# Microtelecom/libperseus-sdr

Hardware: AMD Instinct MI355X
Metric: input MS/s through unpack+decimate, 1/2/4/8 GPU; % HBM-roofline (higher is better)
Workload: dtype i8xi8->i32, f32 out

## Files before the change

### libperseus-sdr_amd/csrc/ddc_kernels.h

```cpp
#ifndef PDDC_DDC_KERNELS_H
#define PDDC_DDC_KERNELS_H

#include <hip/hip_runtime.h>
#include <stdint.h>

#include <atomic>

namespace pddc {

enum InFmt { IN_PACKED24 = 0, IN_F32C = 1 };

struct Tunables {
    std::atomic<int> fir8_dyn_pct{ -1 };
    std::atomic<int> fir8_chunk{ 0 };
    std::atomic<int> fir8_walk{ -1 };
    std::atomic<int> gen_shape_nt{ 0 }, gen_shape_p{ 0 };
    std::atomic<int> no_firp{ 0 };
    std::atomic<int> firp_packed_p{ 0 };
    std::atomic<int> unpack_blocks{ 512 };
    std::atomic<int> debug{ 0 };
    std::atomic<int> push_three_streams{ 0 }, gang_copy_out{ 0 }, gang_gen_inline{ 0 }, gang_solo{ 0 };
    std::atomic<int> chan_run{ 0 };
    std::atomic<int> wblank_run{ 0 };
    std::atomic<int> wblank_chunk{ 0 };
};
Tunables &tunables();
bool set_tunable(const char *name, int value);
bool get_tunable(const char *name, int *value);

struct NcoArgs {
    unsigned long long n0 = 0;
    uint32_t freg = 0;
    uint32_t phase_off = 0;
    uint32_t freg_hist = 0;
    float    lo_c[8], lo_s[8];
    float    lo_c_hist[8], lo_s_hist[8];
};
void nco_fill_steps(NcoArgs *a);

struct Fir8Stage3 {
    const float *taps = nullptr;
    const void  *hist = nullptr;
    void        *hist_out = nullptr;
    float       *out = nullptr;
    void        *seam = nullptr;
    unsigned    *flags = nullptr;
    long long    n_out = 0;
    int d = 0, ntaps = 0, h = 0;
    int off = 0;
    int g = 0, ng = 0;
    int spl = 0, seglen = 0, sl = 0;
    int padf = 0;
    int seam_stride = 0;
};

struct GenTail {
    const float *in = nullptr;
    const float *hist = nullptr;
    float       *hist_out = nullptr;
    float       *out = nullptr;
    const float *taps = nullptr;
    long long    first = 0, n_out = 0, n_batch = 0;
    int          H = 0, D = 0, ntaps = 0;
    int          span = 0, a = 31;
    int          nblocks = 0;
    unsigned     lds = 0;
    int          kind = 0;
    const float *taps2 = nullptr;
    int          nbq = 0;
};
bool gen_tail_shape(GenTail *t, size_t lds_cap, bool have_taps2);
hipError_t launch_gen_tail(const GenTail &t, hipStream_t s);

struct Fir8Args {
    const void *in;
    const void *hist;
    void       *hist_out;
    float      *out;
    const float *taps_blk;
    const float *taps2_blk = nullptr;
    const void  *hist2 = nullptr;
    void        *hist2_out = nullptr;
    unsigned    *sched = nullptr;
    Fir8Stage3   s3;
    GenTail      tail;
    long long   n_in;
    NcoArgs     nco;
};
static_assert(sizeof(Fir8Args) == 448 && offsetof(Fir8Args, n_in) == 288 && offsetof(Fir8Args, nco) == 296 &&
                  offsetof(Fir8Args, nco.freg) == 304 && offsetof(Fir8Args, nco.lo_c) == 316 &&
                  offsetof(Fir8Args, nco.lo_s_hist) == 412,
              "Fir8Args: n_in, then the NCO record (8 + 12 + 128 bytes, padded to 8)");

constexpr int kFir8ManyMax = 8;
struct Fir8Many {
    Fir8Args a[kFir8ManyMax];
};
static_assert(sizeof(Fir8Many) <= 4000, "Fir8Many must fit the kernel-argument segment");
struct GenTailMany {
    GenTail t[kFir8ManyMax];
};
struct SynthMany {
    void              *dst[kFir8ManyMax];
    unsigned long long byte_offset[kFir8ManyMax];
    uint32_t           seed[kFir8ManyMax];
};
bool fir8_many_supported(int kind, int ntb, int R);
hipError_t launch_fir8_many(int kind, int ntb, int R, bool mix, const Fir8Many &m, int n, hipStream_t s);
hipError_t launch_gen_tail_many(const GenTailMany &m, int n, hipStream_t s);
hipError_t launch_synth_lcg_many(const SynthMany &m, int n, size_t nbytes, hipStream_t s);

constexpr int kFirI8Taps16Len = 128 + 6 * 64;
void fir_i8_taps16(const float *taps, int ntaps, int hist, uint16_t *out );

struct FirI8xArgs {
    const void *in;
    const void *hist;
    void       *hist_out;
    float      *out;
    const void *atab;
    long long   n_in;
    float       scale;
    float       ct[2];
    unsigned long long n0;
    uint32_t    freg, phase_off;
    const float *taps2 = nullptr;
    const void  *hist2 = nullptr;
    void        *hist2_out = nullptr;
    long long    n_out = 0;
    int          in_off = 0;
    int          hist_len = 0;
    const void  *taps16 = nullptr;
    float        two_e = 0.0f;
};
constexpr int kFirI8xTaps2Len = 2 * 68;
struct FirI8xMany {
    FirI8xArgs a[kFir8ManyMax];
};
static_assert(sizeof(FirI8xMany) <= 4000, "FirI8xMany must fit the kernel-argument segment");
int    fir_i8x_mode(int hist, bool mix);
size_t fir_i8x_table_bytes(int hist, bool mix);
bool fir_i8x_build_tables(const float *taps, int ntaps, int hist, bool mix, uint32_t freg, int8_t *tables, float *scale,
                          float ct[2], int *exp2 = nullptr);
constexpr int kFirI8xD10Hist = 64;
bool fir_i8x_d10_build_tables(const float *taps, int ntaps, int delay, uint32_t freg, int8_t *tables, float *scale, float ct[2]);
size_t fir_i8x_d10_table_bytes();
hipError_t launch_fir_i8x_d10(const FirI8xArgs &a, hipStream_t s, int max_blocks = 0, int chunk = 0, int layout = -1);
void fir_i8x_taps2(const float *taps2, int ntaps2, bool mix, uint32_t freg, float *out );
bool fir_i8x_supported(int hist, bool mix, bool fuse2);
hipError_t launch_fir_i8x_many(const FirI8xMany &m, int n, int hist, bool mix, bool fuse2, hipStream_t s, int max_blocks = 0,
                               int chunk = 0, int layout = -1);
hipError_t launch_fir_i8x(const FirI8xArgs &a, int hist, bool mix, bool fuse2, hipStream_t s, int max_blocks = 0, int chunk = 0,
                          int layout = -1 );

constexpr int kFirI8xBankMax = 4;
struct FirI8xBankCh {
    const void *atab;
    float      *out;
    void       *hist_out;
    float       scale;
    float       ct[2];
    int         hist_len;
    unsigned long long n0;
    uint32_t    freg, phase_off;
};
struct FirI8xBank {
    FirI8xArgs   a;
    FirI8xBankCh ch[kFirI8xBankMax];
};
static_assert(sizeof(FirI8xBank) <= 4000, "FirI8xBank must fit the kernel-argument segment");
static_assert(offsetof(FirI8xBankCh, n0) == 40 && sizeof(FirI8xBankCh) == 56, "hist_len sits in what was padding");
hipError_t launch_fir_i8x_bank(const FirI8xBank &b, int nch, int hist, hipStream_t s, int max_blocks = 0, int chunk = 0);
hipError_t launch_fir_i8x_bank_d10(const FirI8xBank &b, int nch, hipStream_t s, int max_blocks = 0, int chunk = 0);

constexpr float kFir8PackedTapScale = 0x1.000002p-31f;

constexpr int fir8_tile_inputs(int R, int NT = 256) { return 4 * NT * R; }
// ... 67 lines not shown
```

### libperseus-sdr_amd/csrc/ddc_kernels.hip

```cpp
#include "ddc_kernels.h"
#include "ddc_dev.h"
#include "ddc_host.h"

#include <algorithm>
#include <cmath>
#include <cstdio>
#include <cstdlib>
#include <cstring>
#include <mutex>

static constexpr int PDDC_PRIO_U = 0, PDDC_PRIO_F = 2;

namespace pddc {

Tunables &tunables()
{
    static Tunables t;
    static std::once_flag once;
    std::call_once(once, [] {
        auto env = [](const char *name, std::atomic<int> &v) {
            if (const char *e = getenv(name))
                v.store(atoi(e));
        };
        auto flag = [](const char *name, std::atomic<int> &v) {
            if (getenv(name))
                v.store(1);
        };
        env("PDDC_FIR8_DYN_PCT", t.fir8_dyn_pct);
        env("PDDC_FIR8_CHUNK", t.fir8_chunk);
        env("PDDC_FIR8_WALK", t.fir8_walk);
        if (const char *e = getenv("PDDC_GEN_SHAPE")) {
            int a = 0, b = 0;
            if (sscanf(e, "%d,%d", &a, &b) == 2) {
                t.gen_shape_nt.store(a);
                t.gen_shape_p.store(b);
            }
        }
        flag("PDDC_NO_FIRP", t.no_firp);
        env("PDDC_FIRP_PACKED_P", t.firp_packed_p);
        env("PDDC_UNPACK_BLOCKS", t.unpack_blocks);
        flag("PDDC_DEBUG", t.debug);
        flag("PDDC_PUSH_THREE_STREAMS", t.push_three_streams);
        flag("PDDC_GANG_COPY_OUT", t.gang_copy_out);
        flag("PDDC_GANG_GEN_INLINE", t.gang_gen_inline);
        flag("PDDC_GANG_SOLO", t.gang_solo);
        env("PDDC_CHAN_RUN", t.chan_run);
        env("PDDC_WBLANK_RUN", t.wblank_run);
        env("PDDC_WBLANK_CHUNK", t.wblank_chunk);
    });
    return t;
}

static std::atomic<int> *tunable_by_name(const char *name)
{
    Tunables &t = tunables();
    const struct {
        const char *n;
        std::atomic<int> *v;
    } tab[] = { { "fir8_dyn_pct", &t.fir8_dyn_pct },   { "fir8_chunk", &t.fir8_chunk },       { "fir8_walk", &t.fir8_walk },
                { "gen_shape_nt", &t.gen_shape_nt },
                { "gen_shape_p", &t.gen_shape_p },     { "no_firp", &t.no_firp },             { "firp_packed_p", &t.firp_packed_p },
                { "unpack_blocks", &t.unpack_blocks }, { "debug", &t.debug },                 { "push_three_streams", &t.push_three_streams },
                { "gang_copy_out", &t.gang_copy_out }, { "gang_gen_inline", &t.gang_gen_inline }, { "gang_solo", &t.gang_solo },
                { "chan_run", &t.chan_run },           { "wblank_run", &t.wblank_run },       { "wblank_chunk", &t.wblank_chunk } };
    if (name)
        for (const auto &e : tab)
            if (!strcmp(e.n, name))
                return e.v;
    return nullptr;
}

bool set_tunable(const char *name, int value)
{
    std::atomic<int> *v = tunable_by_name(name);
    if (v)
        v->store(value);
    return v != nullptr;
}

bool get_tunable(const char *name, int *value)
{
    std::atomic<int> *v = tunable_by_name(name);
    if (v && value)
        *value = v->load();
    return v != nullptr;
}

static constexpr int kFused3MaxChunks = 2048;
static constexpr int kPend3 = 4;

static constexpr float kUnpackScale = 0x1.000002p-31f;


__device__ __forceinline__ void unpack8_msb(const uint32_t (&w)[12], int32_t (&I)[8], int32_t (&Q)[8])
{
#pragma unroll
    for (int h = 0; h < 4; ++h) {
        const uint32_t a = w[3 * h], b = w[3 * h + 1], c = w[3 * h + 2];
        I[2 * h]     = (int32_t)__builtin_amdgcn_perm(a, a, 0x0201000cu);
        Q[2 * h]     = (int32_t)__builtin_amdgcn_perm(b, a, 0x0504030cu);
        I[2 * h + 1] = (int32_t)__builtin_amdgcn_perm(c, b, 0x0403020cu);
        Q[2 * h + 1] = (int32_t)(c & 0xffffff00u);
    }
}

template <typename P>
__device__ __forceinline__ void mix8_lo(float (&xi)[8], float (&xq)[8], float cb, float sb, const P &p)
{
#pragma unroll
    for (int e = 0; e < 8; ++e) {
        const float c = cb * p.lo_c[e] - sb * p.lo_s[e];
        const float s = cb * p.lo_s[e] + sb * p.lo_c[e];
        const float r = xi[e] * c - xq[e] * s;
        const float i = xi[e] * s + xq[e] * c;
        xi[e] = r;
        xq[e] = i;
    }
}

__device__ __forceinline__ void cmul(float &a, float &b, float c, float s)
{
    const float r = a * c - b * s;
    const float i = a * s + b * c;
    a = r;
    b = i;
}

__device__ __forceinline__ f32x2 cmul_pk(f32x2 x, f32x2 p)
{
    f32x2 t, y;
    asm("v_pk_mul_f32 %0, %1, %2 op_sel_hi:[0,1]" : "=v"(t) : "v"(x), "v"(p));
    asm("v_pk_fma_f32 %0, %1, %2, %3 op_sel:[1,1,0] op_sel_hi:[1,0,1] neg_lo:[0,1,0]" : "=v"(y) : "v"(x), "v"(p), "v"(t));
    return y;
}
__device__ __forceinline__ f32x2 cmul_pk_s(f32x2 x, float c, float s)
{
    const f32x2 t = __builtin_shufflevector(x, x, 0, 0) * f32x2{ c, s };
    return __builtin_elementwise_fma(__builtin_shufflevector(x, x, 1, 1), f32x2{ -s, c }, t);
}

__device__ __forceinline__ f32x4 cmul2(f32x4 v, float c, float s)
{
    return f32x4{ v.x * c - v.y * s, v.x * s + v.y * c, v.z * c - v.w * s, v.z * s + v.w * c };
}

template <typename P>
__device__ __forceinline__ void mix8(float (&xi)[8], float (&xq)[8], unsigned long long nabs, const P &p,
                                     uint32_t off = 0u)
{
    float cb, sb;
    nco_lo((uint32_t)nabs * p.freg + off, cb, sb);
    mix8_lo(xi, xq, cb, sb, p);
}

static void lo_steps(uint32_t freg, float *c, float *s)
{
    const double k = 6.283185307179586476925286766559 / 4294967296.0;
    for (int e = 0; e < 8; ++e) {
        const uint32_t ph = (uint32_t)((uint64_t)e * freg);
        c[e] = (float)std::cos(k * (double)ph);
        s[e] = (float)(-std::sin(k * (double)ph));
    }
}

void nco_fill_steps(NcoArgs *a)
{
    lo_steps(a->freg, a->lo_c, a->lo_s);
    lo_steps(a->freg_hist, a->lo_c_hist, a->lo_s_hist);
}

struct UnpackArgs {
    const uint8_t *in;
    void          *out;
    long long      ns;
    unsigned long long n0;
    uint32_t       freg;
    uint32_t       phase_off;
    float          lo_c[8];
    float          lo_s[8];
};

template <bool TO_I32, bool MIX>
__global__ __launch_bounds__(256) void k_unpack24(UnpackArgs p)
{
    __shared__ __attribute__((aligned(16))) uint32_t slabs[4][1024];
    const int lane = threadIdx.x & 63;
    uint32_t *slab = slabs[threadIdx.x >> 6];
    const long long ngroups = (((p.ns + 7) >> 3) + 63) & ~63LL;
    for (long long g = (long long)blockIdx.x * 256 + threadIdx.x; g < ngroups;
         g += (long long)gridDim.x * 256) {
        const long long s0 = g << 3;
        uint32_t w[12];
        if (s0 >= p.ns) {
#pragma unroll
            for (int d = 0; d < 12; ++d)
                w[d] = 0;
        } else if (s0 + 8 <= p.ns) {
            const uint4 *src = reinterpret_cast<const uint4 *>(p.in + s0 * 6);
            const uint4 a = src[0], b = src[1], c = src[2];
            w[0] = a.x; w[1] = a.y; w[2] = a.z;  w[3] = a.w;
            w[4] = b.x; w[5] = b.y; w[6] = b.z;  w[7] = b.w;
            w[8] = c.x; w[9] = c.y; w[10] = c.z; w[11] = c.w;
        } else {
            const long long nb = (p.ns - s0) * 6;
#pragma unroll
            for (int d = 0; d < 12; ++d) {
                uint32_t v = 0;
#pragma unroll
                for (int b = 0; b < 4; ++b)
                    if (4 * d + b < nb)
                        v |= (uint32_t)p.in[s0 * 6 + 4 * d + b] << (8 * b);
                w[d] = v;
            }
        }
        int32_t I[8], Q[8];
        unpack8_msb(w, I, Q);
        uint32_t o[16];
// ... 1669 lines not shown
```

### libperseus-sdr_amd/csrc/ddc_wblank.cpp

```cpp
#include "ddc_wblank.h"
#include "ddc_kernels.h"

#include <new>

using namespace pddc;

struct pddc_wblank {
    int device = 0;
    int B = 0, b = 0, H = 0, W = 0, r = 0, D = 0, TL = 0;
    uint32_t thr16 = 16, flags = 0;
    int ncu = 256;
    PackedCarry in;
    uint8_t *d_tail[3] = { nullptr, nullptr, nullptr };
    uint8_t *d_bits[3] = { nullptr, nullptr, nullptr };
    WbState *d_state[3] = { nullptr, nullptr, nullptr };
    int cur = 0;
    uint64_t *d_sums = nullptr, *d_means = nullptr;
};

static void wb_free(pddc_wblank *w)
{
    w->in.d_tail[0] = w->d_tail[0];
    w->in.d_tail[1] = w->d_tail[1];
    w->in.free();
    hipFree(w->d_tail[2]);
    for (int i = 0; i < 3; ++i) {
        hipFree(w->d_bits[i]);
        hipFree(w->d_state[i]);
    }
    hipFree(w->d_sums);
    hipFree(w->d_means);
    delete w;
}

static int wb_clear(pddc_wblank *w)
{
    WbState st{};
    for (uint64_t &h : st.hist)
        h = kWbNoBlock;
    for (int i = 0; i < 3; ++i) {
        PDDC_HIP_TRY(hipMemset(w->d_tail[i], 0, (size_t)(w->TL + 8) * 6));
        PDDC_HIP_TRY(hipMemset(w->d_bits[i], 0, (size_t)wb_tail_bit_bytes(w->D) + 16));
        PDDC_HIP_TRY(hipMemcpy(w->d_state[i], &st, sizeof st, hipMemcpyHostToDevice));
    }
    w->in.reset();
    w->in.tail_len = (uint64_t)w->TL;
    w->cur = 0;
    return PDDC_OK;
}

static int wb_create(pddc_wblank *w)
{
    PDDC_HIP_TRY(hipSetDevice(w->device));
    int ncu = 0;
    PDDC_HIP_TRY(hipDeviceGetAttribute(&ncu, hipDeviceAttributeMultiprocessorCount, w->device));
    w->ncu = ncu > 0 ? ncu : 256;
    const hipError_t e = w->in.alloc((size_t)w->TL + 8);
    w->d_tail[0] = w->in.d_tail[0];
    w->d_tail[1] = w->in.d_tail[1];
    PDDC_HIP_TRY(e);
    PDDC_HIP_TRY(hipMalloc(&w->d_tail[2], ((size_t)w->TL + 8) * 6));
    for (int i = 0; i < 3; ++i) {
        PDDC_HIP_TRY(hipMalloc(&w->d_bits[i], (size_t)wb_tail_bit_bytes(w->D) + 16));
        PDDC_HIP_TRY(hipMalloc(&w->d_state[i], sizeof(WbState)));
    }
    PDDC_HIP_TRY(hipMalloc(&w->d_sums, wblank_sums_len(w->b) * sizeof(uint64_t)));
    PDDC_HIP_TRY(hipMalloc(&w->d_means, wblank_sums_len(w->b) * sizeof(uint64_t)));
    return wb_clear(w);
}

static long long wb_chunk()
{
    const long long c = tunables().wblank_chunk.load();
    return c > 0 && c + 7 < kWbMaxChunk ? (c + 7) & ~7ll : kWbMaxChunk;
}
static long long wb_forced_run()
{
    const long long v = tunables().wblank_run.load();
    return v > 0 ? (v + kWbTile - 1) / kWbTile * kWbTile : 0;
}
static long long wb_run()
{
    const long long forced = wb_forced_run();
    return forced ? forced : kWbTile;
}

static bool wb_batch_ok(const void *p, size_t nsamples) { return !nsamples || (p && !((uintptr_t)p & 15)); }

extern "C" {

int pddc_wblank_tile_samples(void) { return kWbTile; }

int pddc_wblank_run_samples(void)
{
    const long long forced = wb_forced_run();
    return forced ? (int)(forced < (1ll << 30) ? forced : (1ll << 30)) : kWbTile;
}

int pddc_wblank_delay(const pddc_wblank *w) { return w ? w->D : 0; }

int pddc_wblank_create(pddc_wblank **out, int device, const pddc_wblank_params *params, uint32_t thr16, uint32_t flags)
{
    if (!out)
        return pddc_set_error_(PDDC_EINVAL, "null argument");
    *out = nullptr;
    if (!params)
        return pddc_set_error_(PDDC_EINVAL, "wblank: null params");
    if (!wb_params_ok(params->block, params->history, params->guard, params->ramp_log2))
        return pddc_set_error_(PDDC_EINVAL,
                               "wblank: block %d (a power of two 64 .. 4096), history %d (1 .. 16), guard %d (0 .. 128), "
                               "ramp_log2 %d (0 .. 7), guard + 2^ramp_log2 - 1 at most 255",
                               params->block, params->history, params->guard, params->ramp_log2);
    if (!wb_thr_ok(thr16))
        return pddc_set_error_(PDDC_EINVAL, "wblank: thr16 %u (16 .. 65536)", thr16);
    if (flags & ~PDDC_WB_ON)
        return pddc_set_error_(PDDC_EINVAL, "wblank: unknown flags 0x%x", flags);
    if (const int rc = pddc_check_device_(device))
        return rc;
    pddc_wblank *w = new (std::nothrow) pddc_wblank;
    if (!w)
        return pddc_set_error_(PDDC_ENOMEM, "out of memory");
    w->device = device;
    w->B = params->block;
    w->b = wb_log2_block(w->B);
    w->H = params->history;
    w->W = params->guard;
    w->r = params->ramp_log2;
    w->D = wb_delay(w->W, w->r);
    w->TL = wb_tail_len(w->D);
    w->thr16 = thr16;
    w->flags = flags;
    const int rc = wb_create(w);
    if (rc) {
        wb_free(w);
        return rc;
    }
    *out = w;
    return PDDC_OK;
}

int pddc_wblank_destroy(pddc_wblank *w)
{
    if (!w)
        return PDDC_OK;
    (void)hipSetDevice(w->device);
    (void)hipDeviceSynchronize();
    wb_free(w);
    return PDDC_OK;
}

int pddc_wblank_reset(pddc_wblank *w)
{
    if (!w)
        return pddc_set_error_(PDDC_EINVAL, "null argument");
    PDDC_HIP_TRY(hipSetDevice(w->device));
    PDDC_HIP_TRY(hipDeviceSynchronize());
    return wb_clear(w);
}

int pddc_wblank_set(pddc_wblank *w, uint32_t thr16, uint32_t flags)
{
    if (!w)
        return pddc_set_error_(PDDC_EINVAL, "null argument");
    if (!wb_thr_ok(thr16))
        return pddc_set_error_(PDDC_EINVAL, "wblank: thr16 %u (16 .. 65536)", thr16);
    if (flags & ~PDDC_WB_ON)
        return pddc_set_error_(PDDC_EINVAL, "wblank: unknown flags 0x%x", flags);
    w->thr16 = thr16;
    w->flags = flags;
    return PDDC_OK;
}

int pddc_wblank_process(pddc_wblank *w, const void *d_packed, size_t nsamples, void *d_out, void *stream)
{
    if (!w)
        return pddc_set_error_(PDDC_EINVAL, "null argument");
    if (const int rc = PackedCarry::check(d_packed, nsamples))
        return rc;
    if (!wb_batch_ok(d_out, nsamples))
        return pddc_set_error_(PDDC_EINVAL, "wblank: d_out must be a 16-byte aligned device pointer");
    if (!nsamples)
        return PDDC_OK;
    const uintptr_t i0 = (uintptr_t)d_packed, o0 = (uintptr_t)d_out, bytes = (uintptr_t)nsamples * 6;
    if (i0 < o0 + bytes && o0 < i0 + bytes)
        return pddc_set_error_(PDDC_EINVAL, "wblank: d_out overlaps d_packed (there is no in-place form)");
    PDDC_HIP_TRY(hipSetDevice(w->device));
    hipStream_t st = (hipStream_t)stream;

    PackedCarry in = w->in;
    int src_set = w->cur;
    const long long chunk = wb_chunk();
    for (size_t done = 0; done < nsamples;) {
        const size_t n = nsamples - done < (size_t)chunk ? nsamples - done : (size_t)chunk;
        const uint8_t *src = static_cast<const uint8_t *>(d_packed) + done * 6;
        int dst_set = 0;
        while (dst_set == src_set || dst_set == w->cur)
            ++dst_set;
        in.d_tail[0] = w->d_tail[src_set];
        in.d_tail[1] = w->d_tail[dst_set];
        in.cur = 0;
        const PackedCarry::Plan plan = in.plan(n, w->TL + 8, 8);
        WbArgs a{};
        a.in = in.stream(src);
        a.n = (long long)n;
        a.N = in.samples;
        a.b = w->b, a.H = w->H, a.W = w->W, a.r = w->r, a.D = w->D, a.TL = w->TL;
        a.thr16 = w->thr16;
        a.on = w->flags & PDDC_WB_ON;
        a.st = w->d_state[src_set];
        a.new_st = w->d_state[dst_set];
        a.sums = w->d_sums;
        a.means = w->d_means;
        a.nblocks = (long long)wb_blocks_touched(a.N, n, w->b);
        a.bits = w->d_bits[src_set];
        a.new_bits = w->d_bits[dst_set];
        a.out = static_cast<uint8_t *>(d_out) + done * 6;
        a.run = wb_run();
        a.tile_blocks = (int)((a.n + a.run - 1) / a.run);
        a.carry = in.carry(plan, src);
        PDDC_HIP_TRY(hipMemsetAsync(w->d_sums, 0, (size_t)(a.nblocks + 1) * sizeof(uint64_t), st));
        PDDC_HIP_TRY(launch_wblank_sums(a, 8 * w->ncu, st));
        PDDC_HIP_TRY(launch_wblank_means(a, st));
        PDDC_HIP_TRY(launch_wblank_gate(a, st));
        in.commit(plan, n);
        src_set = dst_set;
        done += n;
    }
    w->in = in;
    w->cur = src_set;
    return PDDC_OK;
}

int pddc_wblank_read(pddc_wblank *w, pddc_wblank_status *host, void *stream)
{
    if (!w || !host)
        return pddc_set_error_(PDDC_EINVAL, "null argument");
    PDDC_HIP_TRY(hipSetDevice(w->device));
    WbState st;
    PDDC_HIP_TRY(hipMemcpyAsync(&st, w->d_state[w->cur], sizeof st, hipMemcpyDeviceToHost, (hipStream_t)stream));
    PDDC_HIP_TRY(hipStreamSynchronize((hipStream_t)stream));
    host->mean = st.mean;
    host->triggers = st.triggers;
    host->blanked = st.blanked;
    host->samples = w->in.samples;
    return PDDC_OK;
}

}
```

### libperseus-sdr_amd/csrc/ddc_wblank.h

```cpp
#ifndef PDDC_DDC_WBLANK_H
#define PDDC_DDC_WBLANK_H

#include "ddc_packed.h"
#include "ddc_wblank_gate.h"

namespace pddc {

static constexpr int kWbTile = 2048;
static constexpr long long kWbMaxChunk = 1ll << 26;

struct WbState {
    uint64_t hist[kWbMaxHistory];
    uint64_t partial;
    uint64_t triggers, blanked;
    uint64_t mean;
};

inline size_t wblank_sums_len(int b) { return (size_t)(kWbMaxChunk >> b) + 8; }

struct WbArgs {
    PackedStream in;
    long long n;
    uint64_t N;
    int b, H, W, r, D, TL;
    uint32_t thr16, on;
    const WbState *st;
    WbState *new_st;
    uint64_t *sums;
    uint64_t *means;
    long long nblocks;
    const uint8_t *bits;
    uint8_t *new_bits;
    uint8_t *out;
    long long run;
    int tile_blocks;
    PackedCarryArgs carry;
};

hipError_t launch_wblank_sums(const WbArgs &a, int max_blocks, hipStream_t s);
hipError_t launch_wblank_means(const WbArgs &a, hipStream_t s);
hipError_t launch_wblank_gate(const WbArgs &a, hipStream_t s);

}
#endif
```

### libperseus-sdr_amd/csrc/ddc_wblank.hip

```cpp
#include "ddc_wblank.h"

namespace pddc {

static constexpr int kWbSpanGroups = (kWbTile + 512) / 8;
static constexpr int kWbTrigWords = (kWbTile + 512) / 32 + 2;

__device__ __forceinline__ uint64_t wb_block_sum(const WbArgs &a, long long j)
{
    if (j < 0)
        return a.H + j >= 0 ? a.st->hist[a.H + j] : kWbNoBlock;
    return a.sums[j] + (j == 0 ? a.st->partial : 0);
}

__device__ __forceinline__ uint64_t wb_block_mean(const WbArgs &a, uint64_t k0, long long i)
{
    if (k0 + (uint64_t)i == 0)
        return 0;
    uint64_t m = kWbNoBlock;
    for (int h = 1; h <= a.H; ++h) {
        const uint64_t s = wb_block_sum(a, i - h);
        m = s < m ? s : m;
    }
    return m >> a.b;
}

__device__ __forceinline__ void wb_group_powers(const u32x4 (&raw)[3], uint64_t (&p)[8])
{
#pragma unroll
    for (int h = 0; h < 4; ++h) {
        PDDC_UNPACK_GROUP_MSB(raw, h, i0, q0, i1, q1);
        p[2 * h] = wb_power(wb_code(i0), wb_code(q0));
        p[2 * h + 1] = wb_power(wb_code(i1), wb_code(q1));
    }
}

__global__ __launch_bounds__(256) void k_wblank_sums(WbArgs a)
{
    const long long off = (long long)wb_block_offset(a.N, a.b);
    const long long w0 = off & ~511ll;
    const long long ngroups = (off - w0 + a.n) >> 3;
    const int L = (1 << (a.b - 3)) < 64 ? (1 << (a.b - 3)) : 64;
    const int lane = threadIdx.x & 63;
    for (long long g0 = (long long)blockIdx.x * 256 + (threadIdx.x & ~63); g0 < ngroups; g0 += (long long)gridDim.x * 256) {
        const long long w = w0 + ((g0 + lane) << 3), u = w - off;
        unsigned long long s = 0;
        if (u >= 0 && u < a.n) {
            u32x4 raw[3];
            a.in.load_group(u + a.TL, raw);
            uint64_t p[8];
            wb_group_powers(raw, p);
#pragma unroll
            for (int j = 0; j < 8; ++j)
                s += p[j];
        }
        for (int m = 1; m < L; m <<= 1)
            s += __shfl_xor(s, m);
        if (!(lane & (L - 1)) && s)
            atomicAdd(reinterpret_cast<unsigned long long *>(a.sums + (w >> a.b)), s);
    }
}

__global__ __launch_bounds__(256) void k_wblank_means(WbArgs a)
{
    const long long off = (long long)wb_block_offset(a.N, a.b);
    const uint64_t k0 = wb_block_of(a.N, a.b);
    const int t = threadIdx.x;
    if (blockIdx.x == gridDim.x - 1) {
        const long long done = (off + a.n) >> a.b;
        if (t < kWbMaxHistory)
            a.new_st->hist[t] = t < a.H ? wb_block_sum(a, done - a.H + t) : kWbNoBlock;
        if (t == 16)
            a.new_st->partial = wb_block_sum(a, done);
        if (t == 17)
            a.new_st->triggers = a.st->triggers;
        if (t == 18)
            a.new_st->blanked = a.st->blanked;
        if (t == 19)
            a.new_st->mean = wb_block_mean(a, k0, done);
        return;
    }
    const long long i = (long long)blockIdx.x * 256 + t;
    if (i < a.nblocks)
        a.means[i] = wb_block_mean(a, k0, i);
}

__global__ __launch_bounds__(256) void k_wblank_gate(WbArgs a)
{
    __shared__ u32x4 s_raw[kWbSpanGroups * 3 + 1];
    __shared__ uint32_t s_trig[kWbTrigWords];
    __shared__ unsigned s_cnt[2];
    const int tid = threadIdx.x;

    if ((int)blockIdx.x >= a.tile_blocks) {
        if ((int)blockIdx.x == a.tile_blocks)
            for (long long v = a.n + 8ll * tid; v < a.TL; v += 8 * 256)
                a.new_bits[(v - a.n) >> 3] = a.bits[v >> 3];
        PDDC_CARRY_TAIL(a.carry, a.tile_blocks)
        return;
    }

    const long long off = (long long)wb_block_offset(a.N, a.b);
    const int delta = a.TL - a.D;
    const int own = a.TL >> 3;
    const int q = (6 * delta) >> 2, rr = (6 * delta) & 3;
    uint8_t *trig_bytes = reinterpret_cast<uint8_t *>(s_trig);
    const uint32_t *raw_words = reinterpret_cast<const uint32_t *>(s_raw);
    unsigned ntrig = 0, nblank = 0;
    for (int i = tid; i < kWbTrigWords; i += 256)
        s_trig[i] = 0;
    if (tid < 2)
        s_cnt[tid] = 0;
    if (tid == 0)
        s_raw[kWbSpanGroups * 3] = u32x4{ 0, 0, 0, 0 };

    const long long r0 = (long long)blockIdx.x * a.run;
    const long long r1 = r0 + a.run < a.n ? r0 + a.run : a.n;
    for (long long t0 = r0; t0 < r1; t0 += kWbTile) {
        u32x4 raw[2][3];
        uint64_t mean[2];
        int kind[2];
#pragma unroll
        for (int s = 0; s < 2; ++s) {
            const int gi = tid + 256 * s;
            const long long v = t0 + 8ll * gi, u = v - a.TL;
            kind[s] = gi >= 256 + own ? -1 : u >= a.n ? 0 : u < 0 ? 1 : 2;
            raw[s][0] = raw[s][1] = raw[s][2] = u32x4{ 0, 0, 0, 0 };
            mean[s] = 0;
            if (kind[s] > 0)
                a.in.load_group(v, raw[s]);
            if (kind[s] == 2)
                mean[s] = a.means[(off + u) >> a.b];
        }
        __syncthreads();
#pragma unroll
        for (int s = 0; s < 2; ++s) {
            if (kind[s] < 0)
                continue;
            const int gi = tid + 256 * s;
            const long long v = t0 + 8ll * gi;
            unsigned byte = 0;
            if (kind[s] == 1) {
                byte = a.bits[v >> 3];
            } else if (kind[s] == 2) {
                uint64_t p[8];
                wb_group_powers(raw[s], p);
#pragma unroll
                for (int j = 0; j < 8; ++j)
                    byte |= wb_trigger(a.on != 0, mean[s], p[j], a.thr16) ? 1u << j : 0u;
                if (gi >= own) {
                    ntrig += __popc(byte);
                    if (v >= a.n)
                        a.new_bits[(v - a.n) >> 3] = (uint8_t)byte;
                }
            }
            trig_bytes[gi] = (uint8_t)byte;
            s_raw[3 * gi] = raw[s][0], s_raw[3 * gi + 1] = raw[s][1], s_raw[3 * gi + 2] = raw[s][2];
        }
        __syncthreads();

        const long long n0 = t0 + 8ll * tid;
        if (n0 < a.n) {
            const int lo = 8 * tid + a.TL - 2 * a.D, hi = 8 * tid + 7 + a.TL;
            uint32_t any = 0;
            for (int wd = lo >> 5; wd <= hi >> 5; ++wd)
                any |= s_trig[wd];

            uint32_t w[13], o[12];
#pragma unroll
            for (int i = 0; i < 13; ++i)
                w[i] = raw_words[12 * tid + q + i];
#pragma unroll
            for (int i = 0; i < 12; ++i)
                o[i] = __builtin_amdgcn_alignbyte(w[i + 1], w[i], rr);

            if (any) {
                int num[8];
#pragma unroll
                for (int j = 0; j < 8; ++j) {
                    const int c = 8 * tid + j + delta;
                    int dist = -1;
                    for (int d = 0; d <= a.D; ++d) {
                        const int i0 = c - d, i1 = c + d;
                        if (((s_trig[i0 >> 5] >> (i0 & 31)) | (s_trig[i1 >> 5] >> (i1 & 31))) & 1u) {
                            dist = d;
                            break;
                        }
                    }
                    num[j] = dist < 0 ? -1 : wb_num(dist, a.W);
                    nblank += dist >= 0 && a.N + (uint64_t)(n0 + j) >= (uint64_t)a.D;
                }
#pragma unroll
                for (int h = 0; h < 4; ++h) {
                    if (num[2 * h] >= 0 || num[2 * h + 1] >= 0) {
                        int32_t i0, q0, i1, q1;
                        unpack2_msb(o[3 * h], o[3 * h + 1], o[3 * h + 2], i0, q0, i1, q1);
                        i0 = wb_code(i0), q0 = wb_code(q0), i1 = wb_code(i1), q1 = wb_code(q1);
                        if (num[2 * h] >= 0)
                            i0 = wb_scale(i0, num[2 * h], a.r), q0 = wb_scale(q0, num[2 * h], a.r);
                        if (num[2 * h + 1] >= 0)
                            i1 = wb_scale(i1, num[2 * h + 1], a.r), q1 = wb_scale(q1, num[2 * h + 1], a.r);
                        wb_pack2(i0, q0, i1, q1, o[3 * h], o[3 * h + 1], o[3 * h + 2]);
                    }
                }
            }
            u32x4 *dst = reinterpret_cast<u32x4 *>(a.out + n0 * 6);
#pragma unroll
            for (int c = 0; c < 3; ++c) {
                u32x4 x;
                x[0] = o[4 * c], x[1] = o[4 * c + 1], x[2] = o[4 * c + 2], x[3] = o[4 * c + 3];
                __builtin_nontemporal_store(x, dst + c);
            }
        }
    }

    if (ntrig)
        atomicAdd(&s_cnt[0], ntrig);
    if (nblank)
        atomicAdd(&s_cnt[1], nblank);
    __syncthreads();
    if (tid == 0 && s_cnt[0])
        atomicAdd(reinterpret_cast<unsigned long long *>(&a.new_st->triggers), (unsigned long long)s_cnt[0]);
    if (tid == 1 && s_cnt[1])
        atomicAdd(reinterpret_cast<unsigned long long *>(&a.new_st->blanked), (unsigned long long)s_cnt[1]);
}

hipError_t launch_wblank_sums(const WbArgs &a, int max_blocks, hipStream_t s)
{
    const long long groups = (a.n + 512) >> 3;
    long long blocks = (groups + 255) / 256;
    blocks = blocks < max_blocks ? blocks : max_blocks;
    hipLaunchKernelGGL(k_wblank_sums, dim3((unsigned)blocks), dim3(256), 0, s, a);
    return hipGetLastError();
}

hipError_t launch_wblank_means(const WbArgs &a, hipStream_t s)
{
    hipLaunchKernelGGL(k_wblank_means, dim3((unsigned)((a.nblocks + 255) / 256 + 1)), dim3(256), 0, s, a);
    return hipGetLastError();
}

hipError_t launch_wblank_gate(const WbArgs &a, hipStream_t s)
{
    hipLaunchKernelGGL(k_wblank_gate, dim3((unsigned)(a.tile_blocks + carry_tail_blocks(a.carry.new_len))), dim3(256), 0, s, a);
    return hipGetLastError();
}

}
```

### libperseus-sdr_amd/csrc/ddc_wblank_gate.h

```cpp
#ifndef PDDC_DDC_WBLANK_GATE_H
#define PDDC_DDC_WBLANK_GATE_H

#include <stdint.h>

#ifdef __HIPCC__
#define PDDC_WB_FN __host__ __device__ inline
#else
#define PDDC_WB_FN inline
#endif

namespace pddc {

static constexpr int kWbMinBlock = 64, kWbMaxBlock = 4096, kWbMaxHistory = 16, kWbMaxGuard = 128, kWbMaxRampLog2 = 7;
static constexpr int kWbMaxDelay = 255;
static constexpr uint32_t kWbMinThr16 = 16, kWbMaxThr16 = 65536;
static constexpr uint64_t kWbNoBlock = ~0ull;

PDDC_WB_FN constexpr int wb_log2_block(int B)
{
    for (int b = 6; b <= 12; ++b)
        if (B == (1 << b))
            return b;
    return -1;
}
PDDC_WB_FN constexpr int wb_ramp(int r) { return (1 << r) - 1; }
PDDC_WB_FN constexpr int wb_delay(int W, int r) { return W + wb_ramp(r); }
PDDC_WB_FN constexpr bool wb_params_ok(int B, int H, int W, int r)
{
    return wb_log2_block(B) >= 0 && H >= 1 && H <= kWbMaxHistory && W >= 0 && W <= kWbMaxGuard && r >= 0 &&
           r <= kWbMaxRampLog2 && wb_delay(W, r) <= kWbMaxDelay;
}
PDDC_WB_FN constexpr bool wb_thr_ok(uint32_t thr16) { return thr16 >= kWbMinThr16 && thr16 <= kWbMaxThr16; }

PDDC_WB_FN constexpr int wb_tail_len(int D) { return (2 * D + 7) & ~7; }
PDDC_WB_FN constexpr int wb_tail_bit_bytes(int D) { return wb_tail_len(D) / 8; }

PDDC_WB_FN constexpr uint64_t wb_block_of(uint64_t m, int b) { return m >> b; }
PDDC_WB_FN constexpr uint64_t wb_block_offset(uint64_t m, int b) { return m & ((1ull << b) - 1); }
PDDC_WB_FN constexpr uint64_t wb_blocks_touched(uint64_t N, uint64_t n, int b)
{
    return n ? ((wb_block_offset(N, b) + n - 1) >> b) + 1 : 0;
}

PDDC_WB_FN constexpr int32_t wb_code(int32_t msb) { return msb >> 8; }
PDDC_WB_FN constexpr uint64_t wb_power(int32_t i, int32_t q)
{
    return (uint64_t)((int64_t)i * i) + (uint64_t)((int64_t)q * q);
}
PDDC_WB_FN constexpr uint64_t wb_limit(uint64_t mean, uint32_t thr16) { return (mean * thr16) >> 4; }
PDDC_WB_FN constexpr bool wb_trigger(bool on, uint64_t mean, uint64_t p, uint32_t thr16)
{
    return on && mean > 0 && p > wb_limit(mean, thr16);
}
PDDC_WB_FN constexpr int wb_num(int dist, int W) { return dist <= W ? 0 : dist - W; }
PDDC_WB_FN constexpr int32_t wb_scale(int32_t v, int num, int r)
{
    const uint32_t mag = v < 0 ? 0u - (uint32_t)v : (uint32_t)v;
    const int32_t s = (int32_t)((mag * (uint32_t)num) >> r);
    return v < 0 ? -s : s;
}
PDDC_WB_FN void wb_pack2(int32_t i0, int32_t q0, int32_t i1, int32_t q1, uint32_t &a, uint32_t &b, uint32_t &c)
{
    const uint32_t ui0 = (uint32_t)i0 & 0xffffffu, uq0 = (uint32_t)q0 & 0xffffffu, ui1 = (uint32_t)i1 & 0xffffffu,
                   uq1 = (uint32_t)q1 & 0xffffffu;
    a = ui0 | (uq0 << 24);
    b = (uq0 >> 8) | (ui1 << 16);
    c = (ui1 >> 16) | (uq1 << 8);
}
PDDC_WB_FN void wb_unpack2_msb(uint32_t a, uint32_t b, uint32_t c, int32_t &i0, int32_t &q0, int32_t &i1, int32_t &q1)
{
    i0 = (int32_t)(a << 8);
    q0 = (int32_t)(((a >> 24) | (b << 8)) << 8);
    i1 = (int32_t)(((b >> 16) | (c << 16)) << 8);
    q1 = (int32_t)(c & 0xffffff00u);
}

}
#endif
```

Measured before the change: 889,900.

## Fuse wideband blanker sums, means and gate into one walking kernel

Adds a single-kernel 'walk' design for the wideband noise blanker. Each workgroup walks a run of tiles and keeps block power sums in a shared-memory ring, recomputing a preamble of history instead of launching separate memset, sums, means and gate kernels. Trigger and blank counts are reduced through a global atomic accumulator, with the last block finalising them. It also adds register prefetch of the next span and a perm-based unaligned load. In exchange it redoes the preamble metering per run and adds a heuristic plan selector, with the old design kept as a fallback.

```diff
diff --git a/libperseus-sdr_amd/csrc/ddc_kernels.h b/libperseus-sdr_amd/csrc/ddc_kernels.h
--- a/libperseus-sdr_amd/csrc/ddc_kernels.h
+++ b/libperseus-sdr_amd/csrc/ddc_kernels.h
@@ -23,6 +23,8 @@
     std::atomic<int> chan_run{ 0 };
     std::atomic<int> wblank_run{ 0 };
     std::atomic<int> wblank_chunk{ 0 };
+    std::atomic<int> wblank_design{ 0 };
+    std::atomic<int> wblank_walk{ 0 };
 };
 Tunables &tunables();
 bool set_tunable(const char *name, int value);
diff --git a/libperseus-sdr_amd/csrc/ddc_kernels.hip b/libperseus-sdr_amd/csrc/ddc_kernels.hip
--- a/libperseus-sdr_amd/csrc/ddc_kernels.hip
+++ b/libperseus-sdr_amd/csrc/ddc_kernels.hip
@@ -47,6 +47,8 @@
         env("PDDC_CHAN_RUN", t.chan_run);
         env("PDDC_WBLANK_RUN", t.wblank_run);
         env("PDDC_WBLANK_CHUNK", t.wblank_chunk);
+        env("PDDC_WBLANK_DESIGN", t.wblank_design);
+        env("PDDC_WBLANK_WALK", t.wblank_walk);
     });
     return t;
 }
@@ -62,7 +64,8 @@
                 { "gen_shape_p", &t.gen_shape_p },     { "no_firp", &t.no_firp },             { "firp_packed_p", &t.firp_packed_p },
                 { "unpack_blocks", &t.unpack_blocks }, { "debug", &t.debug },                 { "push_three_streams", &t.push_three_streams },
                 { "gang_copy_out", &t.gang_copy_out }, { "gang_gen_inline", &t.gang_gen_inline }, { "gang_solo", &t.gang_solo },
-                { "chan_run", &t.chan_run },           { "wblank_run", &t.wblank_run },       { "wblank_chunk", &t.wblank_chunk } };
+                { "chan_run", &t.chan_run },           { "wblank_run", &t.wblank_run },       { "wblank_chunk", &t.wblank_chunk },
+                { "wblank_design", &t.wblank_design }, { "wblank_walk", &t.wblank_walk } };
     if (name)
         for (const auto &e : tab)
             if (!strcmp(e.n, name))
diff --git a/libperseus-sdr_amd/csrc/ddc_wblank.cpp b/libperseus-sdr_amd/csrc/ddc_wblank.cpp
--- a/libperseus-sdr_amd/csrc/ddc_wblank.cpp
+++ b/libperseus-sdr_amd/csrc/ddc_wblank.cpp
@@ -16,6 +16,7 @@
     WbState *d_state[3] = { nullptr, nullptr, nullptr };
     int cur = 0;
     uint64_t *d_sums = nullptr, *d_means = nullptr;
+    unsigned long long *d_acc = nullptr;
 };
 
 static void wb_free(pddc_wblank *w)
@@ -30,6 +31,7 @@
     }
     hipFree(w->d_sums);
     hipFree(w->d_means);
+    hipFree(w->d_acc);
     delete w;
 }
 
@@ -43,6 +45,7 @@
         PDDC_HIP_TRY(hipMemset(w->d_bits[i], 0, (size_t)wb_tail_bit_bytes(w->D) + 16));
         PDDC_HIP_TRY(hipMemcpy(w->d_state[i], &st, sizeof st, hipMemcpyHostToDevice));
     }
+    PDDC_HIP_TRY(hipMemset(w->d_acc, 0, 2 * sizeof(unsigned long long)));
     w->in.reset();
     w->in.tail_len = (uint64_t)w->TL;
     w->cur = 0;
@@ -64,8 +67,7 @@
         PDDC_HIP_TRY(hipMalloc(&w->d_bits[i], (size_t)wb_tail_bit_bytes(w->D) + 16));
         PDDC_HIP_TRY(hipMalloc(&w->d_state[i], sizeof(WbState)));
     }
-    PDDC_HIP_TRY(hipMalloc(&w->d_sums, wblank_sums_len(w->b) * sizeof(uint64_t)));
-    PDDC_HIP_TRY(hipMalloc(&w->d_means, wblank_sums_len(w->b) * sizeof(uint64_t)));
+    PDDC_HIP_TRY(hipMalloc(&w->d_acc, 2 * sizeof(unsigned long long)));
     return wb_clear(w);
 }
 
@@ -83,6 +85,31 @@
 {
     const long long forced = wb_forced_run();
     return forced ? forced : kWbTile;
+}
+
+static constexpr int kWbWalkPreambles = 16, kWbWalkGroupsPerCu = 4, kWbWalkMinTiles = 2, kWbWalkMaxExtra8 = 5;
+struct WbPlan {
+    int design;
+    long long run;
+};
+static long long wb_tiles_up(long long v) { return (v + kWbTile - 1) / kWbTile * kWbTile; }
+static WbPlan wb_plan(const pddc_wblank *w, long long n)
+{
+    const int design = tunables().wblank_design.load();
+    if (design == 1)
+        return { 1, wb_run() };
+    const long long preamble = (long long)w->H * w->B + w->TL;
+    const long long forced = tunables().wblank_walk.load();
+    long long run = wb_tiles_up(kWbWalkPreambles * preamble);
+    const long long fill = n / ((long long)kWbWalkGroupsPerCu * w->ncu) / kWbTile * kWbTile;
+    run = run < fill ? run : fill;
+    run = run > kWbWalkMinTiles * kWbTile ? run : kWbWalkMinTiles * kWbTile;
+    if (forced > 0)
+        run = wb_tiles_up(forced);
+    const long long extra = ((n + run - 1) / run - 1) * (preamble < n ? preamble : n);
+    if (design == 2 || 8 * extra <= kWbWalkMaxExtra8 * n)
+        return { 2, run };
+    return { 1, wb_run() };
 }
 
 static bool wb_batch_ok(const void *p, size_t nsamples) { return !nsamples || (p && !((uintptr_t)p & 15)); }
@@ -209,19 +236,29 @@
         a.on = w->flags & PDDC_WB_ON;
         a.st = w->d_state[src_set];
         a.new_st = w->d_state[dst_set];
-        a.sums = w->d_sums;
-        a.means = w->d_means;
         a.nblocks = (long long)wb_blocks_touched(a.N, n, w->b);
         a.bits = w->d_bits[src_set];
         a.new_bits = w->d_bits[dst_set];
         a.out = static_cast<uint8_t *>(d_out) + done * 6;
-        a.run = wb_run();
+        const WbPlan how = wb_plan(w, a.n);
+        a.run = how.run;
         a.tile_blocks = (int)((a.n + a.run - 1) / a.run);
+        a.acc = w->d_acc;
         a.carry = in.carry(plan, src);
-        PDDC_HIP_TRY(hipMemsetAsync(w->d_sums, 0, (size_t)(a.nblocks + 1) * sizeof(uint64_t), st));
-        PDDC_HIP_TRY(launch_wblank_sums(a, 8 * w->ncu, st));
-        PDDC_HIP_TRY(launch_wblank_means(a, st));
-        PDDC_HIP_TRY(launch_wblank_gate(a, st));
+        if (how.design == 2) {
+            PDDC_HIP_TRY(launch_wblank_walk(a, st));
+        } else {
+            if (!w->d_sums)
+                PDDC_HIP_TRY(hipMalloc(&w->d_sums, wblank_sums_len(w->b) * sizeof(uint64_t)));
+            if (!w->d_means)
+                PDDC_HIP_TRY(hipMalloc(&w->d_means, wblank_sums_len(w->b) * sizeof(uint64_t)));
+            a.sums = w->d_sums;
+            a.means = w->d_means;
+            PDDC_HIP_TRY(hipMemsetAsync(w->d_sums, 0, (size_t)(a.nblocks + 1) * sizeof(uint64_t), st));
+            PDDC_HIP_TRY(launch_wblank_sums(a, 8 * w->ncu, st));
+            PDDC_HIP_TRY(launch_wblank_means(a, st));
+            PDDC_HIP_TRY(launch_wblank_gate(a, st));
+        }
         in.commit(plan, n);
         src_set = dst_set;
         done += n;
diff --git a/libperseus-sdr_amd/csrc/ddc_wblank.h b/libperseus-sdr_amd/csrc/ddc_wblank.h
--- a/libperseus-sdr_amd/csrc/ddc_wblank.h
+++ b/libperseus-sdr_amd/csrc/ddc_wblank.h
@@ -34,12 +34,14 @@
     uint8_t *out;
     long long run;
     int tile_blocks;
+    unsigned long long *acc;
     PackedCarryArgs carry;
 };
 
 hipError_t launch_wblank_sums(const WbArgs &a, int max_blocks, hipStream_t s);
 hipError_t launch_wblank_means(const WbArgs &a, hipStream_t s);
 hipError_t launch_wblank_gate(const WbArgs &a, hipStream_t s);
+hipError_t launch_wblank_walk(const WbArgs &a, hipStream_t s);
 
 }
 #endif
diff --git a/libperseus-sdr_amd/csrc/ddc_wblank.hip b/libperseus-sdr_amd/csrc/ddc_wblank.hip
--- a/libperseus-sdr_amd/csrc/ddc_wblank.hip
+++ b/libperseus-sdr_amd/csrc/ddc_wblank.hip
@@ -1,9 +1,16 @@
 #include "ddc_wblank.h"
+
+#ifndef PDDC_WB_WALK_PREFETCH
+#define PDDC_WB_WALK_PREFETCH 1
+#endif
 
 namespace pddc {
 
 static constexpr int kWbSpanGroups = (kWbTile + 512) / 8;
 static constexpr int kWbTrigWords = (kWbTile + 512) / 32 + 2;
+static constexpr int kWbSpanBlocks = (kWbTile + 512) / kWbMinBlock + 1;
+static_assert(kWbMaxHistory + kWbSpanBlocks <= kWbRing && kWbMaxHistory + 1 + kWbTile / kWbMinBlock + 1 <= kWbRing,
+              "the ring holds a run's first window, and a later tile's with the blocks cleared ahead");
 
 __device__ __forceinline__ uint64_t wb_block_sum(const WbArgs &a, long long j)
 {
@@ -84,7 +91,93 @@
         a.means[i] = wb_block_mean(a, k0, i);
 }
 
-__global__ __launch_bounds__(256) void k_wblank_gate(WbArgs a)
+__device__ __forceinline__ void wb_carry_blocks(const WbArgs &a, int tid)
+{
+    if ((int)blockIdx.x == a.tile_blocks)
+        for (long long v = a.n + 8ll * tid; v < a.TL; v += 8 * 256)
+            a.new_bits[(v - a.n) >> 3] = a.bits[v >> 3];
+    PDDC_CARRY_TAIL(a.carry, a.tile_blocks)
+}
+
+template <bool kChunks>
+__device__ __forceinline__ void wb_gate_tile(const WbArgs &a, const uint32_t *s_trig, const uint32_t *raw_words, int tid,
+                                             long long t0, unsigned &nblank)
+{
+    const int delta = a.TL - a.D;
+    const int q = (6 * delta) >> 2, rr = (6 * delta) & 3;
+    const long long n0 = t0 + 8ll * tid;
+    if (n0 >= a.n)
+        return;
+    const int lo = 8 * tid + a.TL - 2 * a.D, hi = 8 * tid + 7 + a.TL;
+    uint32_t any = 0;
+    for (int wd = lo >> 5; wd <= hi >> 5; ++wd)
+        any |= s_trig[wd];
+
+    uint32_t w[13], o[12];
+    if constexpr (kChunks) {
+        const u32x4 *raw_chunks = reinterpret_cast<const u32x4 *>(raw_words) + 3 * tid + (q >> 2);
+        uint32_t f[16], g[15];
+#pragma unroll
+        for (int c = 0; c < 4; ++c) {
+            const u32x4 x = raw_chunks[c];
+            f[4 * c] = x[0], f[4 * c + 1] = x[1], f[4 * c + 2] = x[2], f[4 * c + 3] = x[3];
+        }
+        const uint32_t by1 = q & 1 ? 0x07060504u : 0x03020100u, by2 = q & 2 ? 0x07060504u : 0x03020100u;
+#pragma unroll
+        for (int i = 0; i < 15; ++i)
+            g[i] = __builtin_amdgcn_perm(f[i + 1], f[i], by1);
+#pragma unroll
+        for (int i = 0; i < 13; ++i)
+            w[i] = __builtin_amdgcn_perm(g[i + 2], g[i], by2);
+    } else {
+#pragma unroll
+        for (int i = 0; i < 13; ++i)
+            w[i] = raw_words[12 * tid + q + i];
+    }
+#pragma unroll
+    for (int i = 0; i < 12; ++i)
+        o[i] = __builtin_amdgcn_alignbyte(w[i + 1], w[i], rr);
+
+    if (any) {
+        int num[8];
+#pragma unroll
+        for (int j = 0; j < 8; ++j) {
+            const int c = 8 * tid + j + delta;
+            int dist = -1;
+            for (int d = 0; d <= a.D; ++d) {
+                const int i0 = c - d, i1 = c + d;
+                if (((s_trig[i0 >> 5] >> (i0 & 31)) | (s_trig[i1 >> 5] >> (i1 & 31))) & 1u) {
+                    dist = d;
+                    break;
+                }
+            }
+            num[j] = dist < 0 ? -1 : wb_num(dist, a.W);
+            nblank += dist >= 0 && a.N + (uint64_t)(n0 + j) >= (uint64_t)a.D;
+        }
+#pragma unroll
+        for (int h = 0; h < 4; ++h) {
+            if (num[2 * h] >= 0 || num[2 * h + 1] >= 0) {
+                int32_t i0, q0, i1, q1;
+                unpack2_msb(o[3 * h], o[3 * h + 1], o[3 * h + 2], i0, q0, i1, q1);
+                i0 = wb_code(i0), q0 = wb_code(q0), i1 = wb_code(i1), q1 = wb_code(q1);
+                if (num[2 * h] >= 0)
+                    i0 = wb_scale(i0, num[2 * h], a.r), q0 = wb_scale(q0, num[2 * h], a.r);
+                if (num[2 * h + 1] >= 0)
+                    i1 = wb_scale(i1, num[2 * h + 1], a.r), q1 = wb_scale(q1, num[2 * h + 1], a.r);
+                wb_pack2(i0, q0, i1, q1, o[3 * h], o[3 * h + 1], o[3 * h + 2]);
+            }
+        }
+    }
+    u32x4 *dst = reinterpret_cast<u32x4 *>(a.out + n0 * 6);
+#pragma unroll
+    for (int c = 0; c < 3; ++c) {
+        u32x4 x;
+        x[0] = o[4 * c], x[1] = o[4 * c + 1], x[2] = o[4 * c + 2], x[3] = o[4 * c + 3];
+        __builtin_nontemporal_store(x, dst + c);
+    }
+}
+
+__global__ __launch_bounds__(256) __attribute__((amdgpu_waves_per_eu(6))) void k_wblank_gate(WbArgs a)
 {
     __shared__ u32x4 s_raw[kWbSpanGroups * 3 + 1];
     __shared__ uint32_t s_trig[kWbTrigWords];
@@ -92,17 +185,12 @@
     const int tid = threadIdx.x;
 
     if ((int)blockIdx.x >= a.tile_blocks) {
-        if ((int)blockIdx.x == a.tile_blocks)
-            for (long long v = a.n + 8ll * tid; v < a.TL; v += 8 * 256)
-                a.new_bits[(v - a.n) >> 3] = a.bits[v >> 3];
-        PDDC_CARRY_TAIL(a.carry, a.tile_blocks)
+        wb_carry_blocks(a, tid);
         return;
     }
 
     const long long off = (long long)wb_block_offset(a.N, a.b);
-    const int delta = a.TL - a.D;
     const int own = a.TL >> 3;
-    const int q = (6 * delta) >> 2, rr = (6 * delta) & 3;
     uint8_t *trig_bytes = reinterpret_cast<uint8_t *>(s_trig);
     const uint32_t *raw_words = reinterpret_cast<const uint32_t *>(s_raw);
     unsigned ntrig = 0, nblank = 0;
@@ -158,59 +246,7 @@
         }
         __syncthreads();
 
-        const long long n0 = t0 + 8ll * tid;
-        if (n0 < a.n) {
-            const int lo = 8 * tid + a.TL - 2 * a.D, hi = 8 * tid + 7 + a.TL;
-            uint32_t any = 0;
-            for (int wd = lo >> 5; wd <= hi >> 5; ++wd)
-                any |= s_trig[wd];
-
-            uint32_t w[13], o[12];
-#pragma unroll
-            for (int i = 0; i < 13; ++i)
-                w[i] = raw_words[12 * tid + q + i];
-#pragma unroll
-            for (int i = 0; i < 12; ++i)
-                o[i] = __builtin_amdgcn_alignbyte(w[i + 1], w[i], rr);
-
-            if (any) {
-                int num[8];
-#pragma unroll
-                for (int j = 0; j < 8; ++j) {
-                    const int c = 8 * tid + j + delta;
-                    int dist = -1;
-                    for (int d = 0; d <= a.D; ++d) {
-                        const int i0 = c - d, i1 = c + d;
-                        if (((s_trig[i0 >> 5] >> (i0 & 31)) | (s_trig[i1 >> 5] >> (i1 & 31))) & 1u) {
-                            dist = d;
-                            break;
-                        }
-                    }
-                    num[j] = dist < 0 ? -1 : wb_num(dist, a.W);
-                    nblank += dist >= 0 && a.N + (uint64_t)(n0 + j) >= (uint64_t)a.D;
-                }
-#pragma unroll
-                for (int h = 0; h < 4; ++h) {
-                    if (num[2 * h] >= 0 || num[2 * h + 1] >= 0) {
-                        int32_t i0, q0, i1, q1;
-                        unpack2_msb(o[3 * h], o[3 * h + 1], o[3 * h + 2], i0, q0, i1, q1);
-                        i0 = wb_code(i0), q0 = wb_code(q0), i1 = wb_code(i1), q1 = wb_code(q1);
-                        if (num[2 * h] >= 0)
-                            i0 = wb_scale(i0, num[2 * h], a.r), q0 = wb_scale(q0, num[2 * h], a.r);
-                        if (num[2 * h + 1] >= 0)
-                            i1 = wb_scale(i1, num[2 * h + 1], a.r), q1 = wb_scale(q1, num[2 * h + 1], a.r);
-                        wb_pack2(i0, q0, i1, q1, o[3 * h], o[3 * h + 1], o[3 * h + 2]);
-                    }
-                }
-            }
-            u32x4 *dst = reinterpret_cast<u32x4 *>(a.out + n0 * 6);
-#pragma unroll
-            for (int c = 0; c < 3; ++c) {
-                u32x4 x;
-                x[0] = o[4 * c], x[1] = o[4 * c + 1], x[2] = o[4 * c + 2], x[3] = o[4 * c + 3];
-                __builtin_nontemporal_store(x, dst + c);
-            }
-        }
+        wb_gate_tile<false>(a, s_trig, raw_words, tid, t0, nblank);
     }
 
     if (ntrig)
@@ -224,6 +260,185 @@
         atomicAdd(reinterpret_cast<unsigned long long *>(&a.new_st->blanked), (unsigned long long)s_cnt[1]);
 }
 
+__device__ __forceinline__ void wb_load_span(const WbArgs &a, long long t0, long long r1, int tid, int own, u32x4 (&raw)[2][3])
+{
+#pragma unroll
+    for (int s = 0; s < 2; ++s) {
+        const int gi = tid + 256 * s;
+        const long long v = t0 + 8ll * gi;
+        raw[s][0] = raw[s][1] = raw[s][2] = u32x4{ 0, 0, 0, 0 };
+        if (t0 < r1 && gi < 256 + own && v - a.TL < a.n)
+            a.in.load_group(v, raw[s]);
+    }
+}
+
+__device__ __forceinline__ void wb_ring_add(unsigned long long *ring, uint64_t k0, long long i, const uint64_t (&p)[8])
+{
+    unsigned long long s = 0;
+#pragma unroll
+    for (int j = 0; j < 8; ++j)
+        s += p[j];
+    if (s)
+        atomicAdd(ring + wb_ring_slot(k0, i), s);
+}
+
+__global__ __launch_bounds__(256) void k_wblank_walk(WbArgs a)
+{
+    __shared__ u32x4 s_raw[kWbSpanGroups * 3 + 1];
+    __shared__ uint32_t s_trig[kWbTrigWords];
+    __shared__ unsigned s_cnt[2];
+    __shared__ unsigned long long s_ring[kWbRing];
+    __shared__ uint64_t s_ref[kWbSpanBlocks];
+    const int tid = threadIdx.x;
+
+    if ((int)blockIdx.x >= a.tile_blocks) {
+        wb_carry_blocks(a, tid);
+        return;
+    }
+
+    const long long off = (long long)wb_block_offset(a.N, a.b);
+    const uint64_t k0 = wb_block_of(a.N, a.b);
+    const int own = a.TL >> 3;
+    uint8_t *trig_bytes = reinterpret_cast<uint8_t *>(s_trig);
+    const uint32_t *raw_words = reinterpret_cast<const uint32_t *>(s_raw);
+    unsigned ntrig = 0, nblank = 0;
+    for (int i = tid; i < kWbTrigWords; i += 256)
+        s_trig[i] = 0;
+    if (tid < 2)
+        s_cnt[tid] = 0;
+    if (tid == 0)
+        s_raw[kWbSpanGroups * 3] = u32x4{ 0, 0, 0, 0 };
+    if (tid < kWbRing)
+        s_ring[tid] = 0;
+
+    const long long r0 = (long long)blockIdx.x * a.run;
+    const long long r1 = r0 + a.run < a.n ? r0 + a.run : a.n;
+    u32x4 raw[2][3];
+    wb_load_span(a, r0, r1, tid, own, raw);
+
+    const long long ifirst = wb_walk_first_block(a.N, a.b, a.TL, r0);
+    __syncthreads();
+    if (tid < a.H && tid >= ifirst)
+        s_ring[wb_ring_slot(k0, tid - a.H)] = a.st->hist[tid];
+    if (tid == 64 && ifirst - a.H <= 0)
+        s_ring[wb_ring_slot(k0, 0)] = a.st->partial;
+    __syncthreads();
+    {
+        const long long m0 = wb_walk_meter_from(a.N, a.b, a.H, a.TL, r0), m1 = r0 > a.TL ? r0 - a.TL : 0;
+        for (long long u = m0 + 8ll * tid; u < m1; u += 2 * kWbTile) {
+            u32x4 pre[2][3];
+            const bool two = u + kWbTile < m1;
+            a.in.load_group(u + a.TL, pre[0]);
+            if (two)
+                a.in.load_group(u + kWbTile + a.TL, pre[1]);
+            uint64_t p[8];
+            wb_group_powers(pre[0], p);
+            wb_ring_add(s_ring, k0, (off + u) >> a.b, p);
+            if (two) {
+                wb_group_powers(pre[1], p);
+                wb_ring_add(s_ring, k0, (off + u + kWbTile) >> a.b, p);
+            }
+        }
+    }
+
+    for (long long t0 = r0; t0 < r1; t0 += kWbTile) {
+        const long long t1 = t0 + kWbTile < a.n ? t0 + kWbTile : a.n;
+        const long long ilo = (off + (t0 > a.TL ? t0 - a.TL : 0)) >> a.b, ihi = (off + t1 - 1) >> a.b;
+        int kind[2];
+        __syncthreads();
+#pragma unroll
+        for (int s = 0; s < 2; ++s) {
+            const int gi = tid + 256 * s;
+            const long long u = t0 + 8ll * gi - a.TL;
+            kind[s] = gi >= 256 + own ? -1 : u >= a.n ? 0 : u < 0 ? 1 : 2;
+            if (kind[s] < 0)
+                continue;
+            if (kind[s] == 2 && wb_walk_adds(gi, own, t0 == r0)) {
+                uint64_t p[8];
+                wb_group_powers(raw[s], p);
+                wb_ring_add(s_ring, k0, (off + u) >> a.b, p);
+            }
+            s_raw[3 * gi] = raw[s][0], s_raw[3 * gi + 1] = raw[s][1], s_raw[3 * gi + 2] = raw[s][2];
+        }
+#if PDDC_WB_WALK_PREFETCH
+        wb_load_span(a, t0 + kWbTile, r1, tid, own, raw);
+#endif
+        __syncthreads();
+        if (tid <= ihi - ilo) {
+            const long long i = ilo + tid;
+            uint64_t m = kWbNoBlock;
+            for (int h = 1; h <= a.H; ++h) {
+                const uint64_t v = s_ring[wb_ring_slot(k0, i - h)];
+                m = v < m ? v : m;
+            }
+            s_ref[tid] = k0 + (uint64_t)i == 0 ? 0 : m >> a.b;
+        }
+        __syncthreads();
+#pragma unroll
+        for (int s = 0; s < 2; ++s) {
+            if (kind[s] < 0)
+                continue;
+            const int gi = tid + 256 * s;
+            const long long v = t0 + 8ll * gi, u = v - a.TL;
+            unsigned byte = 0;
+            if (kind[s] == 1) {
+                byte = a.bits[v >> 3];
+            } else if (kind[s] == 2) {
+                const uint64_t mean = s_ref[((off + u) >> a.b) - ilo];
+                const u32x4 again[3] = { s_raw[3 * gi], s_raw[3 * gi + 1], s_raw[3 * gi + 2] };
+                uint64_t p[8];
+                wb_group_powers(again, p);
+#pragma unroll
+                for (int j = 0; j < 8; ++j)
+                    byte |= wb_trigger(a.on != 0, mean, p[j], a.thr16) ? 1u << j : 0u;
+                if (gi >= own) {
+                    ntrig += __popc(byte);
+                    if (v >= a.n)
+                        a.new_bits[(v - a.n) >> 3] = (uint8_t)byte;
+                }
+            }
+            trig_bytes[gi] = (uint8_t)byte;
+        }
+        __syncthreads();
+        wb_gate_tile<true>(a, s_trig, raw_words, tid, t0, nblank);
+        if (tid < kWbTile / kWbMinBlock)
+            s_ring[wb_ring_slot(k0, ihi + 1 + tid)] = 0;
+#if !PDDC_WB_WALK_PREFETCH
+        wb_load_span(a, t0 + kWbTile, r1, tid, own, raw);
+#endif
+    }
+
+    if (ntrig)
+        atomicAdd(&s_cnt[0], ntrig);
+    if (nblank)
+        atomicAdd(&s_cnt[1], nblank);
+    __syncthreads();
+    if (tid == 0) {
+        const unsigned long long old = atomicAdd(a.acc, (unsigned long long)s_cnt[0] | (unsigned long long)s_cnt[1] << 32);
+        if (atomicAdd(a.acc + 1, 1ull + (old >> 63)) == (unsigned long long)a.tile_blocks - 1) {
+            const unsigned long long both = atomicExch(a.acc, 0ull);
+            a.new_st->triggers = a.st->triggers + (both & 0xffffffffull);
+            a.new_st->blanked = a.st->blanked + (both >> 32);
+            atomicExch(a.acc + 1, 0ull);
+        }
+    }
+    if (r1 == a.n) {
+        const long long done = (off + a.n) >> a.b;
+        if (tid < kWbMaxHistory)
+            a.new_st->hist[tid] = tid < a.H ? s_ring[wb_ring_slot(k0, done - a.H + tid)] : kWbNoBlock;
+        if (tid == 16)
+            a.new_st->partial = s_ring[wb_ring_slot(k0, done)];
+        if (tid == 17) {
+            uint64_t m = kWbNoBlock;
+            for (int h = 1; h <= a.H; ++h) {
+                const uint64_t v = s_ring[wb_ring_slot(k0, done - h)];
+                m = v < m ? v : m;
+            }
+            a.new_st->mean = k0 + (uint64_t)done == 0 ? 0 : m >> a.b;
+        }
+    }
+}
+
 hipError_t launch_wblank_sums(const WbArgs &a, int max_blocks, hipStream_t s)
 {
     const long long groups = (a.n + 512) >> 3;
@@ -245,4 +460,10 @@
     return hipGetLastError();
 }
 
-}
+hipError_t launch_wblank_walk(const WbArgs &a, hipStream_t s)
+{
+    hipLaunchKernelGGL(k_wblank_walk, dim3((unsigned)(a.tile_blocks + carry_tail_blocks(a.carry.new_len))), dim3(256), 0, s, a);
+    return hipGetLastError();
+}
+
+}
diff --git a/libperseus-sdr_amd/csrc/ddc_wblank_gate.h b/libperseus-sdr_amd/csrc/ddc_wblank_gate.h
--- a/libperseus-sdr_amd/csrc/ddc_wblank_gate.h
+++ b/libperseus-sdr_amd/csrc/ddc_wblank_gate.h
@@ -75,5 +75,22 @@
     q1 = (int32_t)(c & 0xffffff00u);
 }
 
+static constexpr int kWbRingLog2 = 6, kWbRing = 1 << kWbRingLog2;
+PDDC_WB_FN constexpr long long wb_walk_first_block(uint64_t N, int b, int TL, long long r0)
+{
+    return (long long)((wb_block_offset(N, b) + (uint64_t)(r0 > TL ? r0 - TL : 0)) >> b);
+}
+PDDC_WB_FN constexpr long long wb_walk_last_block(uint64_t N, int b, long long r1)
+{
+    return (long long)((wb_block_offset(N, b) + (uint64_t)(r1 - 1)) >> b);
+}
+PDDC_WB_FN constexpr long long wb_walk_meter_from(uint64_t N, int b, int H, int TL, long long r0)
+{
+    const long long first = wb_walk_first_block(N, b, TL, r0) - H;
+    return first > 0 ? first * (1ll << b) - (long long)wb_block_offset(N, b) : 0;
+}
+PDDC_WB_FN constexpr int wb_ring_slot(uint64_t k0, long long i) { return (int)((k0 + (uint64_t)i) & (uint64_t)(kWbRing - 1)); }
+PDDC_WB_FN constexpr bool wb_walk_adds(int gi, int own, bool first_tile) { return gi >= own || first_tile; }
+
 }
 #endif
```

Result: no change. 889,900 (median of 2 runs) (-0.0%).
